# Ensembl/WiggleTools

Measured on AMD Instinct MI355X. Metric: genomic bp/s (whole node) for 'mean' over N BigWig tracks, higher is better.
Workload: dtype f64

## Files before the change

### include/wiggletools_amd.h

```cpp
#ifndef WIGGLETOOLS_AMD_H_
#define WIGGLETOOLS_AMD_H_

#include <stdint.h>
#include <stdio.h>

#ifdef __cplusplus
extern "C" {
#endif


typedef char wt_bool;

typedef struct wiggleIterator_st WiggleIterator;
typedef struct multiplexer_st Multiplexer;
typedef struct multiset_st Multiset;

struct wiggleIterator_st {
    char *chrom;
    int start;
    int finish;
    double value;
    void *valuePtr;
    wt_bool done;
    int strand;
// ... 343 lines not shown
    int32_t reserved;
} wtamd_pipe_config;

typedef struct {
    int64_t capacity;
    int64_t *seg_off;
    int32_t *start, *finish;
    float *value32;
    double *value64;
} wtamd_pipe_batch;

typedef struct {
    int64_t n_runs;
    const int32_t *start, *finish;
    const double *value;
    const double *tile;
    const uint8_t *inplay;
    int64_t covered_bp;
    int64_t n_intervals;
    int32_t integ_valid;
    int32_t reserved;
    double integ[6];
} wtamd_pipe_result;

typedef struct {
    int64_t batches, intervals, runs, covered_bp;
    int64_t h2d_bytes, d2h_bytes;
    double kernel_ms;
    double h2d_ms, d2h_ms;
    int32_t delta_batches;
    int32_t n_slots;
    double host_submit_ms;
    double host_wait_ms;
    int64_t bw_sections;
    double bw_decode_ms;
} wtamd_pipe_stats;

int wtamd_pipe_create(const wtamd_pipe_config *cfg, wtamd_pipe **out);
void wtamd_pipe_destroy(wtamd_pipe *);
int wtamd_pipe_acquire(wtamd_pipe *, wtamd_pipe_batch *out);
int wtamd_pipe_grow(wtamd_pipe *, int64_t used, int64_t min_capacity, int want_f64, wtamd_pipe_batch *out);
int wtamd_pipe_put_direct(wtamd_pipe *, int64_t at, int64_t count, const int32_t *start, const int32_t *finish,
                          const float *value);
int wtamd_pipe_submit(wtamd_pipe *, int value_is_f64, int32_t range_lo, int32_t range_hi);
int wtamd_pipe_cancel(wtamd_pipe *);
int wtamd_pipe_collect(wtamd_pipe *, wtamd_pipe_result *out);
int wtamd_pipe_release(wtamd_pipe *);
int wtamd_pipe_set_compress(wtamd_pipe *, int on);
int wtamd_pipe_set_integrate(wtamd_pipe *, int on);
int wtamd_pipe_integrate_modes(const wtamd_pipe *);
int wtamd_pipe_integrate_held(wtamd_pipe *, double *integ);
int wtamd_pipe_in_flight(const wtamd_pipe *);
int wtamd_pipe_get_stats(const wtamd_pipe *, wtamd_pipe_stats *out);

typedef struct {
    int64_t comp_off;
    uint32_t comp_size;
    int32_t track;
    uint32_t leaf_start, leaf_end;
} wtamd_bw_section;

typedef struct {
    uint32_t chrom_id;
    uint32_t chrom_len;
    int32_t box;
    int32_t compressed;
    int32_t clip_lo, clip_hi;
    int32_t first_section;
    int32_t n_sections;
    uint32_t plain_bytes;
    int32_t reserved;
} wtamd_bw_track;

int wtamd_pipe_bw_reserve(wtamd_pipe *, int64_t n_bytes, int64_t n_sections, uint8_t **bytes, wtamd_bw_section **sections);
int wtamd_pipe_submit_bw(wtamd_pipe *, int64_t n_bytes, int64_t n_sections, const wtamd_bw_track *tracks,
                         int32_t range_lo, int32_t range_hi);
int64_t wtamd_pipe_bw_fill_sections(const wtamd_pipe *);
unsigned wtamd_pipe_bw_error(const wtamd_pipe *);
int64_t wtamd_pipe_bw_redone(const wtamd_pipe *);

void *wtamd_host_alloc(size_t bytes);
void wtamd_host_free(void *);
void wtamd_pool_stats(int64_t out[6]);
void wtamd_pool_trim(void);


WiggleIterator *wtamd_ArrayReader(int n_chrom, const char *const *chrom_names, const int64_t *seg_off,
                                  const int32_t *start, const int32_t *finish, const float *value,
                                  double default_value);
WiggleIterator *wtamd_OverlappingArrayReader(int n_chrom, const char *const *chrom_names, const int64_t *seg_off,
                                             const int32_t *start, const int32_t *finish, const float *value,
                                             double default_value);
WiggleIterator *wtamd_CoverageIterator(WiggleIterator *child);
WiggleIterator *wtamd_RegionIterator(int op, WiggleIterator *source, WiggleIterator *mask);

Multiplexer *wtamd_ApplyMultiplexer(WiggleIterator *regions, const int *stats, int count, WiggleIterator *dataset, wt_bool strict);
Multiplexer *wtamd_ProfileMultiplexer(WiggleIterator *regions, int width, WiggleIterator *dataset);
WiggleIterator *wtamd_BinIterator(WiggleIterator *child, int width);
WiggleIterator *wtamd_SmoothIterator(WiggleIterator *child, int width);
typedef struct wtamd_histogram_st wtamd_Histogram;
wtamd_Histogram *wtamd_histogram(WiggleIterator **wigs, int count, int width);
void wtamd_normalize_histogram(wtamd_Histogram *hist);
void wtamd_print_histogram(wtamd_Histogram *hist, FILE *file);
int wtamd_histogram_width(const wtamd_Histogram *hist);
int wtamd_histogram_count(const wtamd_Histogram *hist);
const double *wtamd_histogram_row(const wtamd_Histogram *hist, int row);
void wtamd_histogram_range(const wtamd_Histogram *hist, double *lo_hi2);
void wtamd_destroy_histogram(wtamd_Histogram *hist);
WiggleIterator *wtamd_EnergyIntegrator(WiggleIterator *child, int wavelength);
int wtamd_EnergySpectrum(WiggleIterator *child, int n, const int *wavelengths, double *reim);
WiggleIterator *wtamd_TeeWiggleIterator(WiggleIterator *wi, FILE *out, wt_bool bedGraph, wt_bool holdFire);
void wtamd_toFile(WiggleIterator *wi, char *filename, wt_bool bedGraph, wt_bool holdFire);
void wtamd_toStdout(WiggleIterator *wi, wt_bool bedGraph, wt_bool holdFire);
Multiplexer *wtamd_TeeMultiplexer(Multiplexer *in, FILE *out, wt_bool bedGraph, wt_bool holdFire);
void wtamd_toStdoutMultiplexer(Multiplexer *in, wt_bool bedGraph, wt_bool holdFire);
Multiplexer *wtamd_PasteMultiplexer(Multiplexer *in, FILE *infile, FILE *outfile, wt_bool holdFire);
WiggleIterator *wtamd_BigWiggleReader(const char *path, int box);
int wtamd_BigWiggleReaders(int n, const char *const *paths, int box, WiggleIterator **out);
int wtamd_BigWiggleReader_close(WiggleIterator *wi);
WiggleIterator *wtamd_AUCIntegrator(WiggleIterator *wi);
WiggleIterator *wtamd_MeanIntegrator(WiggleIterator *wi);
WiggleIterator *wtamd_PearsonIntegrator(Multiplexer *multi);
WiggleIterator *wtamd_VarianceIntegrator(WiggleIterator *wi);
WiggleIterator *wtamd_StandardDeviationIntegrator(WiggleIterator *wi);
WiggleIterator *wtamd_CoefficientOfVariationIntegrator(WiggleIterator *wi);
WiggleIterator *wtamd_MaxIntegrator(WiggleIterator *wi);
WiggleIterator *wtamd_MinIntegrator(WiggleIterator *wi);
WiggleIterator *wtamd_SpanIntegrator(WiggleIterator *wi);
int64_t wtamd_iterator_next_block(WiggleIterator *wi, const char **chrom, const int32_t **start,
                                  const int32_t **finish, const double **value);
int wtamd_iterator_compress_output(WiggleIterator *wi, int on);
int wtamd_iterator_pipe_stats(WiggleIterator *wi, wtamd_pipe_stats *out);
int64_t wtamd_drain(WiggleIterator *wi, int64_t *covered_bp, double *value_sum);

typedef struct wtamd_bw wtamd_bw;
int wtamd_bw_open(const char *path, wtamd_bw **out);
void wtamd_bw_close(wtamd_bw *);
int wtamd_bw_n_chrom(const wtamd_bw *);
const char *wtamd_bw_chrom_name(const wtamd_bw *, int i);
uint32_t wtamd_bw_chrom_length(const wtamd_bw *, int i);
int64_t wtamd_bw_read_chrom(wtamd_bw *, const char *chrom, int box, int64_t capacity,
                            int32_t *start, int32_t *finish, float *value);

int64_t wtamd_bw_read_part(wtamd_bw *, const char *chrom, int box, int64_t *cursor, int max_blocks, int32_t lo0, int32_t hi0,
                           int64_t capacity, int32_t *start, int32_t *finish, float *value, int *last);

typedef struct bufferedReaderData_st BufferedReaderData;
void launchBufferedReader(void *(*readFileFunction)(void *), void *f_data, BufferedReaderData **buf_data);
wt_bool pushValuesToBuffer(BufferedReaderData *data, const char *chrom, int start, int finish, double value);
void endBufferedSignal(BufferedReaderData *data);
void killBufferedReader(BufferedReaderData *data);
void BufferedReaderPop(WiggleIterator *wi, BufferedReaderData *data);
int compare_chrom_lengths(const void *A, const void *B);
long long wtamd_bufreader_bulk_entries(void);
WiggleIterator *wtamd_BufferedArrayReader(int n_chrom, const char *const *chrom_names, const int64_t *seg_off,
                                          const int32_t *start, const int32_t *finish, const float *value,
                                          double default_value);

typedef struct wtamd_bw_writer wtamd_bw_writer;
int wtamd_bw_writer_open(const char *path, int n_chrom, const char *const *names, const uint32_t *lengths, int items_per_block,
                         int zlib_level, wtamd_bw_writer **out);
int wtamd_bw_writer_add(wtamd_bw_writer *, int chrom, int64_t n, const int32_t *start, const int32_t *finish, const float *value);
int64_t wtamd_bw_writer_close(wtamd_bw_writer *);
int wtamd_bw_writers_add_chrom(wtamd_bw_writer *const *writers, int n_tracks, int chrom, const int64_t *seg_off, const int32_t *start,
                               const int32_t *finish, const float *value, int threads);

// ... 13 lines not shown
```

### wiggletools_amd/csrc/wt_engine.hip

```cpp
#include <hip/hip_runtime.h>

#include <cstdio>
#include <thread>
#include <atomic>
#include <cstring>
#include <map>
#include <mutex>
#include <string>
#include <vector>

#include "wt_host.h"
#include "wt_trackset.h"
#include "wt_core.h"
#include "wt_plan.h"
#include "wt_kernels.h"
#include "wt_devscope.h"
#include "wt_pool.h"

#ifndef WT_INDEX_UNROLL
#define WT_INDEX_UNROLL 2
#endif
#define WT_INDEX_CHUNK (256 * 4 * WT_INDEX_UNROLL)
__global__ void __launch_bounds__(256) wt_index_kernel(const WtParams P, long long total, long long span) {
    const long long dev_total = P.seg_off[(long long) P.n_chrom * P.n_tracks];
// ... 169 lines not shown
    for (long long q = t; q < n_status; q += stride) status[q] = 0ull;
    for (long long q = t; q < n_counters; q += stride) counters[q] = 0ull;
    for (long long q = t; q < n_cro; q += stride) chrom_run_off[q] = 0;
}

__global__ void __launch_bounds__(256) wt_validate_kernel(const int32_t *start, const int32_t *finish, const int64_t *seg_off,
                                                           long long n_seg, long long total, unsigned long long *out) {
    const long long g = (long long) blockIdx.x * blockDim.x + threadIdx.x;
    if (g >= total) return;
    bool bad = finish[g] <= start[g];
    if (!bad && g > 0 && start[g] < finish[g - 1]) {
        long long lo = 0, hi = n_seg;
        while (hi - lo > 1) {
            const long long mid = (lo + hi) >> 1;
            if (seg_off[mid] <= g) lo = mid; else hi = mid;
        }
        bad = seg_off[lo] != g;
    }
    if (bad) {
        atomicAdd(&out[0], 1ull);
        atomicMin(&out[1], (unsigned long long) g);
    }
}

static thread_local std::string g_last_error;

int wt_fail(int code, const std::string &msg) {
    g_last_error = msg;
    return code;
}

template <class T>
static hipError_t wt_grow(T **p, int64_t *cap, int64_t need, bool *quiet) {
    if (*cap >= need && *p) return hipSuccess;
    int64_t c = *cap * 2;
    if (c < need) c = need;
    if (c < 1) c = 1;
    if (*p) {
        if (!*quiet) {
            const hipError_t eq = wt_pool_quiesce();
            if (eq != hipSuccess) return eq;
            *quiet = true;
        }
        (void) wt_dev_free(*p);
    }
    *p = nullptr; *cap = 0;
    const hipError_t e = wt_dev_alloc(p, sizeof(T) * (size_t) c);
    if (e == hipSuccess) *cap = c;
    return e;
}

static void wt_free_windows(WtWindows &w) {
    (void) wt_dev_free(w.d_tabs);
    (void) wt_dev_free(w.d_widx); (void) wt_dev_free(w.d_cidx); (void) wt_dev_free(w.d_status); (void) wt_dev_free(w.d_bad_list); (void) wt_dev_free(w.d_bad_goff);
    if (w.h_tab) wt_host_free(w.h_tab);
    if (w.ev_tab) (void) hipEventDestroy(w.ev_tab);
    w = WtWindows();
}

extern "C" {

const char *wtamd_last_error(void) { return g_last_error.c_str(); }
const char *wtamd_version(void) { return "wiggletools_amd 0.1 (gfx950)"; }

int wtamd_device_count(void) {
    int n = 0;
    if (hipGetDeviceCount(&n) != hipSuccess) return 0;
    return n;
}

__global__ void wt_warm_kernel(int *p) { if (p && threadIdx.x == 4096) *p = 0; }

static std::mutex g_warm_mu;
static std::thread *g_warm_thread = nullptr;
static bool g_warm_started = false;

extern "C++" void wt_warmup_join() {
    std::thread *t = nullptr;
    { std::lock_guard<std::mutex> lk(g_warm_mu); t = g_warm_thread; g_warm_thread = nullptr; }
    if (t) { t->join(); delete t; }
}

static std::atomic<int> g_device_chosen{-1};

void wtamd_warmup_async(void) {
    std::lock_guard<std::mutex> lk(g_warm_mu);
    if (g_warm_started || getenv("WTAMD_NO_WARMUP")) return;
    int n = 0, cur = -1;
    if (hipGetDeviceCount(&n) != hipSuccess || n <= 0) { (void) hipGetLastError(); return; }
    int ordinal = g_device_chosen.load();
    if (ordinal < 0 && hipGetDevice(&cur) == hipSuccess && (n == 1 || cur > 0)) ordinal = cur;
    if (ordinal < 0 || ordinal >= n) return;
    g_warm_started = true;
    g_warm_thread = new std::thread([ordinal] {
        if (hipSetDevice(ordinal) != hipSuccess) { (void) hipGetLastError(); return; }
        hipStream_t st[3] = {nullptr, nullptr, nullptr};
        for (auto &s : st)
            if (hipStreamCreateWithFlags(&s, hipStreamNonBlocking) != hipSuccess) s = nullptr;
        for (auto &s : st)
            if (s) hipLaunchKernelGGL(wt_warm_kernel, dim3(1), dim3(64), 0, s, (int *) nullptr);
        for (auto &s : st)
            if (s) { (void) hipStreamSynchronize(s); (void) hipStreamDestroy(s); }
        (void) hipGetLastError();
    });
    atexit(wt_warmup_join);
}

int wtamd_set_device(int ordinal) {
    wt_warmup_join();
    WT_HIP(hipSetDevice(ordinal));
    g_device_chosen.store(ordinal);
    return WTAMD_OK;
}

int wtamd_current_device(void) {
    int d = 0;
    if (hipGetDevice(&d) != hipSuccess) { (void) hipGetLastError(); return -1; }
    return d;
}

extern "C++" int wt_trackset_common(const wtamd_tracks *t, wtamd_trackset *ts) {
    if (!t || t->n_chrom < 0 || t->n_tracks <= 0 || !t->seg_off || !t->defaults)
        return wt_fail(WTAMD_ERR_ARG, "wtamd_trackset_create: bad tracks descriptor");
    if (wtamd_device_count() <= 0) return wt_fail(WTAMD_ERR_NODEVICE, "no HIP device visible");
    ts->n_chrom = t->n_chrom;
    ts->n_tracks = t->n_tracks;
    ts->value_f64 = t->value_is_f64 != 0;
    const int64_t n_seg = (int64_t) t->n_chrom * t->n_tracks;
    ts->seg_off.assign(t->seg_off, t->seg_off + n_seg + 1);
    for (int64_t s = 0; s < n_seg; s++)
        if (ts->seg_off[s + 1] < ts->seg_off[s]) return wt_fail(WTAMD_ERR_ARG, "seg_off not monotone");
    ts->n_intervals = ts->seg_off[n_seg] - ts->seg_off[0];
    if (ts->seg_off[0] != 0) return wt_fail(WTAMD_ERR_ARG, "seg_off[0] must be 0");
    ts->defaults.assign(t->defaults, t->defaults + t->n_tracks);
    if (t->range_lo && t->range_hi) {
        ts->range_lo.assign(t->range_lo, t->range_lo + t->n_chrom);
        ts->range_hi.assign(t->range_hi, t->range_hi + t->n_chrom);
    }
    ts->scratch_f32 = !ts->value_f64 && wt_defaults_fit_f32(ts->defaults.data(), ts->n_tracks);
    WT_HIP(hipGetDevice(&ts->device));
    hipDeviceProp_t prop;
    WT_HIP(hipGetDeviceProperties(&prop, ts->device));
    ts->num_cu = prop.multiProcessorCount;
    WT_HIP(wt_dev_alloc(&ts->d_seg_off, sizeof(int64_t) * (n_seg + 1)));
    WT_HIP(hipMemcpy(ts->d_seg_off, ts->seg_off.data(), sizeof(int64_t) * (n_seg + 1), hipMemcpyHostToDevice));
    WT_HIP(wt_dev_alloc(&ts->d_defaults, sizeof(double) * t->n_tracks));
    WT_HIP(hipMemcpy(ts->d_defaults, ts->defaults.data(), sizeof(double) * t->n_tracks, hipMemcpyHostToDevice));
    WT_HIP(wt_dev_alloc(&ts->d_counters, sizeof(unsigned long long) * WT_CTR_N));
    WT_HIP(wt_host_alloc((void **) &ts->h_counters, sizeof(unsigned long long) * WT_CTR_N));
    WT_HIP(wt_host_alloc((void **) &ts->h_debug, sizeof(unsigned long long) * 16));
    memset(ts->h_debug, 0, sizeof(unsigned long long) * 16);
    WT_HIP(wt_dev_alloc(&ts->d_chrom_run_off, sizeof(int64_t) * (t->n_chrom + 1)));
    WT_HIP(hipEventCreate(&ts->ev_i0));
    WT_HIP(hipEventCreate(&ts->ev_i1));
    WT_HIP(hipEventCreate(&ts->ev_r0));
    WT_HIP(hipEventCreate(&ts->ev_r1));
    return WTAMD_OK;
}

extern "C++" int wt_check_extents(wtamd_trackset *ts) {
    for (size_t q = 0; q < ts->last_finish.size(); q++)
        if (ts->seg_off[q + 1] > ts->seg_off[q] && ts->last_finish[q] > WTAMD_MAX_COORD) {
            const int64_t bad = ts->last_finish[q];
            return wt_fail(WTAMD_ERR_ARG, "run finish " + std::to_string(bad) + " above the supported maximum " +
                           std::to_string((long long) WTAMD_MAX_COORD) + " (2^31 - 65537)");
        }
    return WTAMD_OK;
}

static int wt_refresh_extents_device(wtamd_trackset *ts, hipStream_t s) {
    const int64_t n_seg = (int64_t) ts->n_chrom * ts->n_tracks;
    ts->first_start.assign(n_seg, 0);
    ts->last_finish.assign(n_seg, 0);
    if (n_seg > 0 && ts->n_intervals > 0) {
        const size_t bytes = sizeof(int32_t) * 2 * (size_t) n_seg;
        if (!ts->d_extents) WT_HIP(wt_dev_alloc(&ts->d_extents, bytes));
        if (!ts->h_extents) WT_HIP(wt_host_alloc((void **) &ts->h_extents, bytes));
        hipLaunchKernelGGL(wt_extents_kernel, dim3((unsigned) ((n_seg + 255) / 256)), dim3(256), 0, s,
                           ts->d_seg_off, ts->d_start, ts->d_finish, (long long) n_seg, ts->d_extents, ts->d_extents + n_seg);
        WT_HIP(hipGetLastError());
        WT_HIP(hipMemcpyAsync(ts->h_extents, ts->d_extents, bytes, hipMemcpyDeviceToHost, s));
        WT_HIP(hipStreamSynchronize(s));
        ts->first_start.assign(ts->h_extents, ts->h_extents + n_seg);
        ts->last_finish.assign(ts->h_extents + n_seg, ts->h_extents + 2 * n_seg);
    }
    return WTAMD_OK;
}

static int wt_create_host_impl(const wtamd_tracks *t, wtamd_trackset *ts) {
    int rc = wt_trackset_common(t, ts);
    if (rc != WTAMD_OK) return rc;
    ts->owns = true;
    const int64_t n = ts->n_intervals;
    const size_t vsz = ts->value_f64 ? 8 : 4;
    const int64_t n_alloc = n > 0 ? n : 1;
    WT_HIP(hipMalloc(&ts->d_start, sizeof(int32_t) * n_alloc));
    WT_HIP(hipMalloc(&ts->d_finish, sizeof(int32_t) * n_alloc));
    WT_HIP(hipMalloc(&ts->d_value, vsz * n_alloc));
    if (n > 0) {
        if (!t->start || !t->finish || !t->value) return wt_fail(WTAMD_ERR_ARG, "NULL arrays");
        WT_HIP(hipMemcpy(ts->d_start, t->start, sizeof(int32_t) * n, hipMemcpyHostToDevice));
        WT_HIP(hipMemcpy(ts->d_finish, t->finish, sizeof(int32_t) * n, hipMemcpyHostToDevice));
        WT_HIP(hipMemcpy(ts->d_value, t->value, vsz * n, hipMemcpyHostToDevice));
    }
    const int64_t n_seg = (int64_t) ts->n_chrom * ts->n_tracks;
    ts->first_start.assign(n_seg, 0);
    ts->last_finish.assign(n_seg, 0);
    for (int64_t s = 0; s < n_seg; s++)
        if (ts->seg_off[s + 1] > ts->seg_off[s]) {
            ts->first_start[s] = t->start[ts->seg_off[s]];
            ts->last_finish[s] = t->finish[ts->seg_off[s + 1] - 1];
        }
    return wt_check_extents(ts);
}

int wtamd_trackset_create_host(const wtamd_tracks *t, wtamd_trackset **out) {
    if (!out) return wt_fail(WTAMD_ERR_ARG, "out == NULL");
    wtamd_trackset *ts = new wtamd_trackset();
    const int rc = wt_create_host_impl(t, ts);
    if (rc != WTAMD_OK) { wtamd_trackset_destroy(ts); return rc; }
    *out = ts;
    return WTAMD_OK;
}

static int wt_create_device_impl(const wtamd_tracks *t, wtamd_trackset *ts) {
    int rc = wt_trackset_common(t, ts);
    if (rc != WTAMD_OK) return rc;
    ts->owns = false;
    ts->d_start = const_cast<int32_t *>(t->start);
    ts->d_finish = const_cast<int32_t *>(t->finish);
    ts->d_value = const_cast<void *>(t->value);
    rc = wt_refresh_extents_device(ts, nullptr);
    if (rc != WTAMD_OK) return rc;
    return wt_check_extents(ts);
}

int wtamd_trackset_create_device(const wtamd_tracks *t, wtamd_trackset **out) {
    if (!out) return wt_fail(WTAMD_ERR_ARG, "out == NULL");
    wtamd_trackset *ts = new wtamd_trackset();
    const int rc = wt_create_device_impl(t, ts);
    if (rc != WTAMD_OK) { wtamd_trackset_destroy(ts); return rc; }
    *out = ts;
    return WTAMD_OK;
}

void wtamd_trackset_destroy(wtamd_trackset *ts) {
    if (!ts) return;
    (void) wt_pool_quiesce();
    if (ts->owns) { (void) hipFree(ts->d_start); (void) hipFree(ts->d_finish); (void) hipFree(ts->d_value); }
    (void) wt_dev_free(ts->d_seg_off); (void) wt_dev_free(ts->d_defaults); (void) wt_dev_free(ts->d_counters); (void) wt_dev_free(ts->d_chrom_run_off);
    (void) wt_dev_free(ts->d_extents);
    (void) hipFree(ts->d_gscratch); (void) hipFree(ts->d_mwu_table);
    for (double *q : ts->mwu_retired) (void) hipFree(q);
    if (ts->h_counters) wt_host_free(ts->h_counters);
    if (ts->h_debug) wt_host_free(ts->h_debug);
    if (ts->h_extents) wt_host_free(ts->h_extents);
    for (auto &kv : ts->windows) wt_free_windows(kv.second);
    if (ts->ev_i0) (void) hipEventDestroy(ts->ev_i0);
    if (ts->ev_i1) (void) hipEventDestroy(ts->ev_i1);
    if (ts->ev_r0) (void) hipEventDestroy(ts->ev_r0);
    if (ts->ev_r1) (void) hipEventDestroy(ts->ev_r1);
    delete ts;
}

static int64_t wt_span(const wtamd_trackset *ts) {
    int64_t span = 0;
    for (int c = 0; c < ts->n_chrom; c++) {
        int64_t lo = INT64_MAX, hi = INT64_MIN;
        for (int i = 0; i < ts->n_tracks; i++) {
            const int64_t s = (int64_t) c * ts->n_tracks + i;
            if (ts->seg_off[s + 1] > ts->seg_off[s]) {
                lo = std::min<int64_t>(lo, ts->first_start[s]);
                hi = std::max<int64_t>(hi, ts->last_finish[s]);
            }
        }
        if (lo <= hi) span += hi - lo;
    }
    return span;
}

int64_t wtamd_trackset_max_runs(const wtamd_trackset *ts) {
    if (!ts) return 0;
    return std::min<int64_t>(2 * ts->n_intervals, wt_span(ts));
}

static int wt_get_windows(wtamd_trackset *ts, int W, WtWindows **out, hipStream_t s = nullptr) {
    WtWindows &w = ts->windows[W];
    *out = &w;
    if (w.tab_valid) return WTAMD_OK;
    wt_make_windows(ts->n_chrom, ts->n_tracks, ts->seg_off.data(), ts->first_start.data(), ts->last_finish.data(), W, w.tab,
                    ts->range_lo.empty() ? nullptr : ts->range_lo.data(),
                    ts->range_hi.empty() ? nullptr : ts->range_hi.data(), false);
    w.indexed = false;
    const int64_t nc = ts->n_chrom > 0 ? ts->n_chrom : 1;
    const int64_t nwin = w.tab.n_windows > 0 ? w.tab.n_windows : 1;
    const int64_t nwidx = (w.tab.n_rows > 0 ? w.tab.n_rows : 1) * (int64_t) ts->n_tracks;
    auto up8 = [](int64_t x) { return (x + 7) & ~(int64_t) 7; };
    bool quiet = false;
    if (w.cap_chrom < nc || w.cap_win < nwin || !w.d_tabs) {
        const int64_t cc = w.cap_chrom < nc ? std::max<int64_t>(nc, 2 * w.cap_chrom) : w.cap_chrom;
        const int64_t cw = w.cap_win < nwin ? std::max<int64_t>(nwin, 2 * w.cap_win) : w.cap_win;
        const int64_t o_cnwin = up8(4 * cc), o_chi = o_cnwin + up8(4 * cc), o_cfirst = o_chi + up8(4 * cc), o_win = o_cfirst + 8 * (cc + 1);
        const int64_t total = o_win + up8(4 * cw);
        if (w.d_tabs || w.d_status) { WT_HIP(wt_pool_quiesce()); quiet = true; }
        (void) wt_dev_free(w.d_tabs);
        w.d_tabs = nullptr; w.cap_tabs = 0;
        w.d_cbase = w.d_cnwin = w.d_chi = w.d_win_chrom = nullptr; w.d_cfirst = nullptr;
        if (w.cap_win < cw) { (void) wt_dev_free(w.d_status); w.d_status = nullptr; }
        w.cap_chrom = 0; w.cap_win = 0;
        WT_HIP(wt_dev_alloc(&w.d_tabs, (size_t) total));
        if (!w.d_status) WT_HIP(wt_dev_alloc(&w.d_status, sizeof(unsigned long long) * (size_t) cw));
        w.cap_tabs = total;
        w.d_cbase = (int32_t *) w.d_tabs; w.d_cnwin = (int32_t *) (w.d_tabs + o_cnwin); w.d_chi = (int32_t *) (w.d_tabs + o_chi);
        w.d_cfirst = (int64_t *) (w.d_tabs + o_cfirst); w.d_win_chrom = (int32_t *) (w.d_tabs + o_win);
        w.cap_chrom = cc; w.cap_win = cw;
    }
    WT_HIP(wt_grow(&w.d_widx, &w.cap_widx, nwidx, &quiet));
    WT_HIP(wt_grow(&w.d_cidx, &w.cap_cidx, ((w.tab.n_rows > 0 ? w.tab.n_rows : 1) + WT_ISEARCH_ROWS - 1) / WT_ISEARCH_ROWS * (int64_t) ts->n_tracks, &quiet));
    if (ts->n_chrom > 0) {
        if (ts->pipe_mode && ts->n_chrom != 1) return wt_fail(WTAMD_ERR_INTERNAL, "pipeline slots hold one chromosome");
        if (!w.ev_tab) WT_HIP(hipEventCreateWithFlags(&w.ev_tab, hipEventDisableTiming));
        if (w.tab_in_flight) { WT_HIP(hipEventSynchronize(w.ev_tab)); w.tab_in_flight = false; }
        const int64_t head = (char *) w.d_win_chrom - w.d_tabs;
        if (w.h_tab_bytes < head) {
            if (w.h_tab) wt_host_free(w.h_tab);
            w.h_tab = nullptr; w.h_tab_bytes = 0;
            WT_HIP(wt_host_alloc((void **) &w.h_tab, (size_t) head));
            w.h_tab_bytes = head;
        }
        const int64_t o_cfirst = (char *) w.d_cfirst - w.d_tabs;
        const int64_t used = o_cfirst + (int64_t) sizeof(int64_t) * (ts->n_chrom + 1);
        memset(w.h_tab, 0, (size_t) used);
        memcpy(w.h_tab + ((char *) w.d_cbase - w.d_tabs), w.tab.cbase.data(), sizeof(int32_t) * ts->n_chrom);
        memcpy(w.h_tab + ((char *) w.d_cnwin - w.d_tabs), w.tab.c_nwin.data(), sizeof(int32_t) * ts->n_chrom);
        memcpy(w.h_tab + ((char *) w.d_chi - w.d_tabs), w.tab.c_hi.data(), sizeof(int32_t) * ts->n_chrom);
        memcpy(w.h_tab + o_cfirst, w.tab.c_first_win.data(), sizeof(int64_t) * (ts->n_chrom + 1));
        WT_HIP(hipMemcpyAsync(w.d_tabs, w.h_tab, (size_t) used, hipMemcpyHostToDevice, s));
        WT_HIP(hipEventRecord(w.ev_tab, s));
        w.tab_in_flight = true;
        if (w.tab.n_windows > 0) {
            if (ts->n_chrom == 1) {
                WT_HIP(hipMemsetAsync(w.d_win_chrom, 0, sizeof(int32_t) * (size_t) w.tab.n_windows, s));
            } else {
                hipLaunchKernelGGL(wt_win_chrom_kernel, dim3((unsigned) ((w.tab.n_windows + 255) / 256)), dim3(256), 0, s,
                                   (const int64_t *) w.d_cfirst, ts->n_chrom, (long long) w.tab.n_windows, w.d_win_chrom);
                WT_HIP(hipGetLastError());
            }
        }
    }
    w.tab_valid = true;
    return WTAMD_OK;
}

static void wt_fill_params(const wtamd_trackset *ts, const WtWindows *w, const WtPlan &plan, WtParams &P) {
    memset(&P, 0, sizeof(P));
    P.start = ts->d_start; P.finish = ts->d_finish; P.value = ts->d_value;
    P.seg_off = ts->d_seg_off; P.defaults = ts->d_defaults;
    P.n_chrom = ts->n_chrom; P.n_tracks = ts->n_tracks; P.n_total = ts->n_intervals;
    P.cbase = w->d_cbase; P.c_nwin = w->d_cnwin; P.c_hi = w->d_chi; P.c_first_win = w->d_cfirst;
    P.n_windows = w->tab.n_windows; P.win_chrom = w->d_win_chrom; P.widx = w->d_widx;
    P.status = w->d_status; P.counters = ts->d_counters; P.debug = ts->h_debug;
    wt_plan_to_params(plan, P);
}

static int wt_build_index(wtamd_trackset *ts, WtWindows *w, const WtPlan &plan, hipStream_t s) {
    WtParams P;
    wt_fill_params(ts, w, plan, P);
    WT_HIP(hipEventRecord(ts->ev_i0, s));
    static const int mode = [] {
        const char *e = getenv("WTAMD_INDEX"), *c = getenv("WTAMD_INDEX_CHECK");
        if (c && atoi(c) > 0) return 2;
        return (e && !strcmp(e, "scan")) ? 1 : 0;
    }();
    const size_t n_widx = (size_t) w->tab.n_rows * ts->n_tracks;
    auto scan = [&](uint32_t *dst) -> int {
        WtParams Q = P;
        Q.widx = dst;
        WT_HIP(hipMemsetAsync(dst, 0, sizeof(uint32_t) * n_widx, s));
        if (ts->n_intervals > 0) {
            const long long total = ts->n_intervals;
            long long blocks = (total + WT_INDEX_CHUNK - 1) / WT_INDEX_CHUNK;
            const long long cap = (long long) ts->num_cu * 8;
            if (blocks > cap) blocks = cap;
            long long span = (total + blocks - 1) / blocks;
            span = (span + WT_INDEX_CHUNK - 1) / WT_INDEX_CHUNK * WT_INDEX_CHUNK;
            blocks = (total + span - 1) / span;
            hipLaunchKernelGGL(wt_index_kernel, dim3((unsigned) blocks), dim3(256), 0, s, Q, total, span);
            WT_HIP(hipGetLastError());
        }
        return WTAMD_OK;
    };
    auto search = [&](uint32_t *dst) -> int {
        WtParams Q = P;
        Q.widx = dst;
        const long long n_rows = w->tab.n_rows;
        if (n_rows > 0 && ts->n_tracks > 0) {
            const long long n_strips = (n_rows + WT_ISEARCH_ROWS - 1) / WT_ISEARCH_ROWS;
            if (w->cap_cidx < n_strips * ts->n_tracks) return wt_fail(WTAMD_ERR_INTERNAL, "coarse window index not allocated");
            hipLaunchKernelGGL(wt_index_coarse_kernel, dim3((unsigned) ((n_strips * ts->n_tracks + 255) / 256)), dim3(256), 0, s, Q, n_strips, w->d_cidx);
            WT_HIP(hipGetLastError());
            const dim3 grid((unsigned) n_strips, (unsigned) ((ts->n_tracks + WT_ISEARCH_TRACKS - 1) / WT_ISEARCH_TRACKS));
            hipLaunchKernelGGL(wt_index_search_kernel, grid, dim3(WT_ISEARCH_ROWS * WT_ISEARCH_TRACKS), 0, s, Q, n_rows, n_strips, (const uint32_t *) w->d_cidx);
            WT_HIP(hipGetLastError());
        }
        return WTAMD_OK;
    };
    if (mode == 1) {
        if (int rc = scan(w->d_widx)) return rc;
    } else {
        if (int rc = search(w->d_widx)) return rc;
    }
    if (mode == 2 && n_widx > 0) {
        uint32_t *other = nullptr;
        unsigned long long *d_diff = nullptr, h_diff = 0;
        WT_HIP(hipMalloc(&other, sizeof(uint32_t) * n_widx));
        WT_HIP(hipMalloc(&d_diff, sizeof(unsigned long long)));
        WT_HIP(hipMemsetAsync(d_diff, 0, sizeof(unsigned long long), s));
        if (int rc = scan(other)) return rc;
        hipLaunchKernelGGL(wt_index_compare_kernel, dim3((unsigned) ((n_widx + 255) / 256)), dim3(256), 0, s, w->d_widx, other, (long long) n_widx, d_diff);
        WT_HIP(hipMemcpyAsync(&h_diff, d_diff, sizeof(h_diff), hipMemcpyDeviceToHost, s));
        WT_HIP(hipStreamSynchronize(s));
        (void) hipFree(other); (void) hipFree(d_diff);
        if (h_diff) {
            fprintf(stderr, "wiggletools_amd: WTAMD_INDEX_CHECK: the searched window index differs from the scanned one in %llu of %zu entries\n", h_diff, n_widx);
            return wt_fail(WTAMD_ERR_INTERNAL, "window index check failed");
        }
    }
    WT_HIP(hipEventRecord(ts->ev_i1, s));
    ts->have_index_time = true;
    w->indexed = true;
    return WTAMD_OK;
}

static inline int wt_delta_class(int op) { return op == WT_OP_TTEST ? 1 : ((op == WT_OP_MAX || op == WT_OP_MIN) ? 2 : 0); }
static bool wt_wants_delta(const wtamd_trackset *ts, int op) {
    return !ts->delta_failed_[wt_delta_class(op)] && wt_delta_eligible(op, ts->value_f64, ts->n_tracks, ts->defaults.data());
}

static double wt_events_per_bp(const wtamd_trackset *ts) {
    const int64_t span = wt_span(ts);
    return span > 0 ? 1.25 * (double) ts->n_intervals / (double) span : 0.0;
}

static bool wt_mwu_few_ties(wtamd_trackset *ts, hipStream_t stream) {
    if (ts->mwu_few_ties >= 0) return ts->mwu_few_ties != 0;
    ts->mwu_few_ties = 0;
    if (hipStreamSynchronize(stream) != hipSuccess) { (void) hipGetLastError(); return false; }
    const int64_t n = ts->n_intervals;
    if (n < 1024 || ts->value_f64 || !ts->d_value) return false;
    const int64_t S = std::min<int64_t>(4096, n), stride = n / S;
    std::vector<uint32_t> v((size_t) S);
    if (hipMemcpy2D(v.data(), 4, ts->d_value, (size_t) stride * 4, 4, (size_t) S, hipMemcpyDeviceToHost) != hipSuccess) { (void) hipGetLastError(); return false; }
    std::sort(v.begin(), v.end());
    const int64_t distinct = (int64_t) (std::unique(v.begin(), v.end()) - v.begin());
    ts->mwu_few_ties = distinct * 100 >= S * 97 ? 1 : 0;
    return ts->mwu_few_ties != 0;
}

static bool wt_pick_plan(wtamd_trackset *ts, int op, int n_set0, WtPlan &plan, std::string &err, hipStream_t stream = nullptr) {
    static const int mwalk = getenv("WTAMD_MWALK") ? (atoi(getenv("WTAMD_MWALK")) != 0 ? 1 : 0) : -1;
    const bool walk = !getenv("WTAMD_NO_WALK");
    const bool mwu_walk = op == WT_OP_MWU && mwalk != 0 && !ts->value_f64 && walk && (mwalk == 1 || wt_mwu_few_ties(ts, stream));
    const double events_per_bp = (op == WT_OP_MEDIAN || op == WT_OP_MWU) ? wt_events_per_bp(ts) : 0.0;
    return wt_pick_general_plan(ts->n_tracks, op, ts->value_f64, ts->scratch_f32, n_set0, walk, mwu_walk, events_per_bp, plan, err);
}

static void wt_trackset_forget(wtamd_trackset *ts, bool delta_failed) {
    for (int q = 0; q < 3; q++) { ts->delta_verified_[q] = false; ts->delta_failed_[q] = delta_failed; ts->delta_n_bad_[q] = 0; }
    for (auto &kv : ts->windows) kv.second.indexed = false;
}

extern "C++" int wt_trackset_rebind(wtamd_trackset *ts, int64_t n, const int64_t *seg_off, int32_t range_lo, int32_t range_hi, bool value_f64,
                                    int32_t *d_start, int32_t *d_finish, void *d_value, bool delta_failed) {
    ts->n_intervals = n;
    ts->seg_off.assign(seg_off, seg_off + (int64_t) ts->n_chrom * ts->n_tracks + 1);
    ts->range_lo[0] = range_lo;
    ts->range_hi[0] = range_hi;
    ts->value_f64 = value_f64;
    ts->scratch_f32 = !ts->value_f64 && wt_defaults_fit_f32(ts->defaults.data(), ts->n_tracks);
    ts->d_start = d_start; ts->d_finish = d_finish; ts->d_value = d_value;
    wt_trackset_forget(ts, delta_failed);
    for (auto &kv : ts->windows) kv.second.tab_valid = false;
    return wt_check_extents(ts);
}

int wtamd_trackset_index(wtamd_trackset *ts, int op, void *stream) {
    if (!ts) return wt_fail(WTAMD_ERR_ARG, "ts == NULL");
    wt_trackset_forget(ts, false);
    ts->mwu_few_ties = -1;
    if (!ts->owns && !ts->pipe_mode) {
        int rce = wt_refresh_extents_device(ts, (hipStream_t) stream);
        if (rce != WTAMD_OK) return rce;
        rce = wt_check_extents(ts);
        if (rce != WTAMD_OK) return rce;
        for (auto &kv : ts->windows) kv.second.tab_valid = false;
    }
    WtPlan plan;
    std::string err;
    if (wt_wants_delta(ts, op)) wt_make_delta_plan_for(plan, ts->n_tracks, op);
    else if (!wt_pick_plan(ts, op, ts->n_tracks / 2, plan, err, (hipStream_t) stream)) return wt_fail(WTAMD_ERR_ARG, err);
    WtWindows *w = nullptr;
    int rc = wt_get_windows(ts, plan.W, &w, (hipStream_t) stream);
    if (rc != WTAMD_OK) return rc;
    return wt_build_index(ts, w, plan, (hipStream_t) stream);
}

extern "C++" int wt_check_desc(const wtamd_trackset *ts, const wtamd_reduce_desc *d) {
    if (!ts || !d) return wt_fail(WTAMD_ERR_ARG, "NULL argument");
    if (d->op < 0 || d->op >= WTAMD_OP_COUNT_) return wt_fail(WTAMD_ERR_ARG, "unknown op");
    if (d->op == WTAMD_OP_TTEST) {
        if (d->n_set0 < 3 || ts->n_tracks - d->n_set0 < 3)
            return wt_fail(WTAMD_ERR_ARG, "The t-test function only works for two sets with enough elements to compute variance");
    } else if (d->op == WTAMD_OP_MWU) {
        if (d->n_set0 < 1 || ts->n_tracks - d->n_set0 < 1)
            return wt_fail(WTAMD_ERR_ARG, "The Mann-Whitney U function only works for two non-empty sets");
    }
    return WTAMD_OK;
}

static int wt_reduce_plan(wtamd_trackset *ts, const WtPlan &plan, int op, uint32_t flags, int n_set0, wtamd_runs *runs,
                          double *d_tile, uint8_t *d_inplay, int64_t *n_runs, hipStream_t s);

extern "C++" int wt_launch_patch(wtamd_trackset *ts, int delta_W, int op, uint32_t flags, int n_set0, wtamd_runs *runs, long long n_bad,
                                 hipStream_t s) {
    WtPlan plan;
    std::string err;
    if (!wt_make_plan(ts->n_tracks, op, ts->scratch_f32, plan, err)) return wt_fail(WTAMD_ERR_INTERNAL, err);
    if (!wt_patch_compatible(plan, delta_W, ts->scratch_f32, ts->value_f64))
        return wt_fail(WTAMD_ERR_INTERNAL, "no general plan compatible with the difference-array windows (general W " + std::to_string(plan.W) + ", difference-array W " +
                       std::to_string(delta_W) + ", slab " + std::to_string((long long) plan.scratch_slab) + ", float staging " + std::to_string((int) ts->scratch_f32) + ", f64 values " +
                       std::to_string((int) ts->value_f64) + ")");
    WtWindows *dw = nullptr, *w = nullptr;
    int rc = wt_get_windows(ts, delta_W, &dw, s);
    if (rc != WTAMD_OK) return rc;
    rc = wt_get_windows(ts, plan.W, &w, s);
    if (rc != WTAMD_OK) return rc;
    WtLaunch L;
    WtParams &P = L.P;
    wt_fill_params(ts, w, plan, P);
    P.op = op; P.flags = flags; P.n_set0 = op == WT_OP_TTEST ? n_set0 : 0;
    P.capacity = runs->capacity;
    P.o_start = runs->start; P.o_finish = runs->finish; P.o_value = runs->value;
    P.chrom_run_off = runs->chrom_run_off ? runs->chrom_run_off : ts->d_chrom_run_off;
    L.T = plan.T; L.lds = plan.lds_bytes; L.stream = s; L.num_cu = ts->num_cu;
    WtPatchArgs Q;
    Q.bad_list = dw->d_bad_list; Q.bad_goff = dw->d_bad_goff;
    Q.n_bad = ts->d_counters + WT_CTR_DELTA_BAD;
    Q.d_win_chrom = dw->d_win_chrom; Q.d_c_first_win = dw->d_cfirst;
    Q.ratio = delta_W / plan.W;
    if (!wt_patch_launch(L, Q, op, plan.ppt, plan.n_chunks > 1, n_bad, !w->indexed))
        return wt_fail(WTAMD_ERR_INTERNAL, "no general plan compatible with the difference-array windows");
    if (L.err != hipSuccess) return wt_fail(WTAMD_ERR_HIP, std::string("patch kernel launch: ") + hipGetErrorString(L.err));
    WT_HIP(hipEventRecord(ts->ev_r1, s));
    ts->stats.patched_windows = (int32_t) n_bad;
    return WTAMD_OK;
}

static int wt_reduce_impl(wtamd_trackset *ts, int op, uint32_t flags, int n_set0, wtamd_runs *runs,
                          double *d_tile, uint8_t *d_inplay, int64_t *n_runs, hipStream_t s) {
    if (!runs || !runs->start || !runs->finish || !runs->value)
        return wt_fail(WTAMD_ERR_ARG, "wtamd_reduce: output arrays missing");
    WtPlan plan;
    std::string err;
    if (!d_tile && wt_wants_delta(ts, op)) {
        wt_make_delta_plan_for(plan, ts->n_tracks, op);
        const int dc = wt_delta_class(op);
        int64_t n_probe = 0;
        const bool probe = !ts->delta_verified_[dc];
        const int rc = wt_reduce_plan(ts, plan, op, flags, n_set0, runs, d_tile, d_inplay,
                                      (probe && !n_runs) ? &n_probe : n_runs, s);
        if (!probe) {
            if (ts->delta_n_bad_[dc] > 0 && (rc == WTAMD_OK || rc == WTAMD_ERR_CAPACITY)) {
                const int rp = wt_launch_patch(ts, plan.W, op, flags, n_set0, runs, ts->delta_n_bad_[dc], s);
                if (rp != WTAMD_OK) return rp;
                if (n_runs) WT_HIP(hipStreamSynchronize(s));
            }
            return rc;
        }
        if (rc != WTAMD_OK && rc != WTAMD_ERR_CAPACITY) return rc;
        const long long n_bad = (long long) ts->h_counters[WT_CTR_DELTA_BAD];
        if (n_bad == 0) { ts->delta_verified_[dc] = true; ts->delta_n_bad_[dc] = 0; return rc; }
        if (wt_few_enough_to_patch(n_bad, ts->stats.n_windows) && !getenv("WTAMD_NO_PATCH")) {
            const int rp = wt_launch_patch(ts, plan.W, op, flags, n_set0, runs, n_bad, s);
            if (rp == WTAMD_OK) {
                WT_HIP(hipStreamSynchronize(s));
                ts->delta_verified_[dc] = true;
                ts->delta_n_bad_[dc] = n_bad;
// ... 322 lines not shown
```

### wiggletools_amd/csrc/wt_trackset.h

```cpp
#ifndef WT_TRACKSET_H_
#define WT_TRACKSET_H_

#include <map>
#include <vector>

#include "wt_host.h"
#include "wt_plan.h"

struct WtWindows {
    WtPlan plan_geom;
    WtWindowTables tab;
    int32_t *d_cbase = nullptr, *d_cnwin = nullptr, *d_chi = nullptr, *d_win_chrom = nullptr;
    int64_t *d_cfirst = nullptr;
    uint32_t *d_widx = nullptr;
    uint32_t *d_cidx = nullptr;
    unsigned long long *d_status = nullptr;
    int32_t *d_bad_list = nullptr;
    long long *d_bad_goff = nullptr;
    bool indexed = false;
    int64_t cap_chrom = 0, cap_win = 0, cap_widx = 0, cap_bad = 0, cap_cidx = 0;
    bool tab_valid = false;
    char *h_tab = nullptr;
    int64_t h_tab_bytes = 0;
    hipEvent_t ev_tab = nullptr;
    bool tab_in_flight = false;
    char *d_tabs = nullptr;
    int64_t cap_tabs = 0;
};

struct wtamd_trackset {
    int n_chrom = 0, n_tracks = 0;
    bool value_f64 = false;
    bool owns = false;
    int64_t n_intervals = 0;
    std::vector<int64_t> seg_off;
    std::vector<double> defaults;
    std::vector<int32_t> first_start, last_finish;
    std::vector<int32_t> range_lo, range_hi;
    int32_t *d_start = nullptr, *d_finish = nullptr;
    void *d_value = nullptr;
    int64_t *d_seg_off = nullptr;
    double *d_defaults = nullptr;
    unsigned long long *d_counters = nullptr;
    unsigned long long *h_counters = nullptr;
    unsigned long long *h_debug = nullptr;
    int64_t *d_chrom_run_off = nullptr;
    int32_t *d_extents = nullptr, *h_extents = nullptr;
    char *d_gscratch = nullptr;
    size_t gscratch_bytes = 0;
    double *d_mwu_table = nullptr;
    int mwu_n1 = -1, mwu_n2 = -1, mwu_kmax = 0;
    int mwu_few_ties = -1;
    std::vector<double *> mwu_retired;
    std::map<int, WtWindows> windows;
    hipEvent_t ev_i0 = nullptr, ev_i1 = nullptr, ev_r0 = nullptr, ev_r1 = nullptr;
    bool have_index_time = false, have_reduce_time = false;
    wtamd_stats stats{};
    int device = 0;
    int num_cu = 256;
    bool scratch_f32 = false;
    bool delta_failed_[3] = {false, false, false};
    bool delta_verified_[3] = {false, false, false};
    long long delta_n_bad_[3] = {0, 0, 0};
    bool pipe_mode = false;
};

void wt_warmup_join();
int wt_trackset_common(const wtamd_tracks *t, wtamd_trackset *ts);
int wt_check_extents(wtamd_trackset *ts);
int wt_check_desc(const wtamd_trackset *ts, const wtamd_reduce_desc *d);

int wt_trackset_rebind(wtamd_trackset *ts, int64_t n, const int64_t *seg_off, int32_t range_lo, int32_t range_hi, bool value_f64,
                       int32_t *d_start, int32_t *d_finish, void *d_value, bool delta_failed);

int wt_reduce_enqueue(wtamd_trackset *ts, const wtamd_reduce_desc &desc, wtamd_runs *runs, double *d_tile, uint8_t *d_inplay,
                      hipStream_t s, bool *used_delta, int *delta_W);

int wt_launch_patch(wtamd_trackset *ts, int delta_W, int op, uint32_t flags, int n_set0, wtamd_runs *runs, long long n_bad,
                    hipStream_t s);

int wt_multiplex_device(wtamd_trackset *ts, uint32_t flags, wtamd_runs *runs, double *d_tile, uint8_t *d_inplay, int64_t *n_runs,
                        hipStream_t s);

#endif
```

Baseline: 50.45 billion.

## Speculatively build window index while device extents readback is in flight

The index build no longer blocks on a stream synchronize after the extents kernel. It records an event, picks the plan and enqueues the window and index build using the previous extents, then waits. If the fresh extents match the previous ones the speculative index is kept; otherwise it is invalidated and rebuilt. It also drops the single-chromosome memset shortcut in favour of always launching the win_chrom kernel, and adds counters for kept and redone indexes. When extents change, the speculative work is wasted and the index is built twice.

```diff
diff --git a/include/wiggletools_amd.h b/include/wiggletools_amd.h
--- a/include/wiggletools_amd.h
+++ b/include/wiggletools_amd.h
@@ -449,6 +449,7 @@
 void *wtamd_host_alloc(size_t bytes);
 void wtamd_host_free(void *);
 void wtamd_pool_stats(int64_t out[6]);
+void wtamd_index_stats(int64_t out[2]);
 void wtamd_pool_trim(void);
 
 
diff --git a/wiggletools_amd/csrc/wt_engine.hip b/wiggletools_amd/csrc/wt_engine.hip
--- a/wiggletools_amd/csrc/wt_engine.hip
+++ b/wiggletools_amd/csrc/wt_engine.hip
@@ -275,6 +275,7 @@
 }
 
 static std::atomic<int> g_device_chosen{-1};
+static std::atomic<int64_t> g_index_kept{0}, g_index_redone{0};
 
 void wtamd_warmup_async(void) {
     std::lock_guard<std::mutex> lk(g_warm_mu);
@@ -348,23 +349,29 @@
     WT_HIP(hipEventCreate(&ts->ev_i1));
     WT_HIP(hipEventCreate(&ts->ev_r0));
     WT_HIP(hipEventCreate(&ts->ev_r1));
-    return WTAMD_OK;
+    WT_HIP(hipEventCreateWithFlags(&ts->ev_ext, hipEventDisableTiming));
+    return WTAMD_OK;
+}
+
+static int64_t wt_first_bad_extent(const wtamd_trackset *ts) {
+    for (size_t q = 0; q < ts->last_finish.size(); q++)
+        if (ts->seg_off[q + 1] > ts->seg_off[q] && ts->last_finish[q] > WTAMD_MAX_COORD) return (int64_t) q;
+    return -1;
 }
 
 extern "C++" int wt_check_extents(wtamd_trackset *ts) {
-    for (size_t q = 0; q < ts->last_finish.size(); q++)
-        if (ts->seg_off[q + 1] > ts->seg_off[q] && ts->last_finish[q] > WTAMD_MAX_COORD) {
-            const int64_t bad = ts->last_finish[q];
-            return wt_fail(WTAMD_ERR_ARG, "run finish " + std::to_string(bad) + " above the supported maximum " +
-                           std::to_string((long long) WTAMD_MAX_COORD) + " (2^31 - 65537)");
-        }
-    return WTAMD_OK;
-}
-
-static int wt_refresh_extents_device(wtamd_trackset *ts, hipStream_t s) {
+    const int64_t q = wt_first_bad_extent(ts);
+    if (q >= 0) {
+        const int64_t bad = ts->last_finish[q];
+        return wt_fail(WTAMD_ERR_ARG, "run finish " + std::to_string(bad) + " above the supported maximum " +
+                       std::to_string((long long) WTAMD_MAX_COORD) + " (2^31 - 65537)");
+    }
+    return WTAMD_OK;
+}
+
+static int wt_extents_enqueue(wtamd_trackset *ts, hipStream_t s, bool *pending) {
     const int64_t n_seg = (int64_t) ts->n_chrom * ts->n_tracks;
-    ts->first_start.assign(n_seg, 0);
-    ts->last_finish.assign(n_seg, 0);
+    *pending = false;
     if (n_seg > 0 && ts->n_intervals > 0) {
         const size_t bytes = sizeof(int32_t) * 2 * (size_t) n_seg;
         if (!ts->d_extents) WT_HIP(wt_dev_alloc(&ts->d_extents, bytes));
@@ -373,10 +380,35 @@
                            ts->d_seg_off, ts->d_start, ts->d_finish, (long long) n_seg, ts->d_extents, ts->d_extents + n_seg);
         WT_HIP(hipGetLastError());
         WT_HIP(hipMemcpyAsync(ts->h_extents, ts->d_extents, bytes, hipMemcpyDeviceToHost, s));
-        WT_HIP(hipStreamSynchronize(s));
+        WT_HIP(hipEventRecord(ts->ev_ext, s));
+        *pending = true;
+    }
+    return WTAMD_OK;
+}
+
+static bool wt_extents_same(const wtamd_trackset *ts) {
+    const size_t n_seg = (size_t) ts->n_chrom * ts->n_tracks;
+    return ts->first_start.size() == n_seg && ts->last_finish.size() == n_seg &&
+           !memcmp(ts->h_extents, ts->first_start.data(), sizeof(int32_t) * n_seg) &&
+           !memcmp(ts->h_extents + n_seg, ts->last_finish.data(), sizeof(int32_t) * n_seg);
+}
+
+static void wt_extents_adopt(wtamd_trackset *ts, bool pending) {
+    const int64_t n_seg = (int64_t) ts->n_chrom * ts->n_tracks;
+    ts->first_start.assign(n_seg, 0);
+    ts->last_finish.assign(n_seg, 0);
+    if (pending) {
         ts->first_start.assign(ts->h_extents, ts->h_extents + n_seg);
         ts->last_finish.assign(ts->h_extents + n_seg, ts->h_extents + 2 * n_seg);
     }
+}
+
+static int wt_refresh_extents_device(wtamd_trackset *ts, hipStream_t s) {
+    bool pending = false;
+    const int rc = wt_extents_enqueue(ts, s, &pending);
+    if (rc != WTAMD_OK) return rc;
+    if (pending) WT_HIP(hipStreamSynchronize(s));
+    wt_extents_adopt(ts, pending);
     return WTAMD_OK;
 }
 
@@ -453,6 +485,7 @@
     if (ts->ev_i1) (void) hipEventDestroy(ts->ev_i1);
     if (ts->ev_r0) (void) hipEventDestroy(ts->ev_r0);
     if (ts->ev_r1) (void) hipEventDestroy(ts->ev_r1);
+    if (ts->ev_ext) (void) hipEventDestroy(ts->ev_ext);
     delete ts;
 }
 
@@ -532,13 +565,9 @@
         WT_HIP(hipEventRecord(w.ev_tab, s));
         w.tab_in_flight = true;
         if (w.tab.n_windows > 0) {
-            if (ts->n_chrom == 1) {
-                WT_HIP(hipMemsetAsync(w.d_win_chrom, 0, sizeof(int32_t) * (size_t) w.tab.n_windows, s));
-            } else {
-                hipLaunchKernelGGL(wt_win_chrom_kernel, dim3((unsigned) ((w.tab.n_windows + 255) / 256)), dim3(256), 0, s,
-                                   (const int64_t *) w.d_cfirst, ts->n_chrom, (long long) w.tab.n_windows, w.d_win_chrom);
-                WT_HIP(hipGetLastError());
-            }
+            hipLaunchKernelGGL(wt_win_chrom_kernel, dim3((unsigned) ((w.tab.n_windows + 255) / 256)), dim3(256), 0, s,
+                               (const int64_t *) w.d_cfirst, ts->n_chrom, (long long) w.tab.n_windows, w.d_win_chrom);
+            WT_HIP(hipGetLastError());
         }
     }
     w.tab_valid = true;
@@ -681,21 +710,53 @@
     if (!ts) return wt_fail(WTAMD_ERR_ARG, "ts == NULL");
     wt_trackset_forget(ts, false);
     ts->mwu_few_ties = -1;
-    if (!ts->owns && !ts->pipe_mode) {
-        int rce = wt_refresh_extents_device(ts, (hipStream_t) stream);
-        if (rce != WTAMD_OK) return rce;
-        rce = wt_check_extents(ts);
-        if (rce != WTAMD_OK) return rce;
-        for (auto &kv : ts->windows) kv.second.tab_valid = false;
-    }
+    const hipStream_t s = (hipStream_t) stream;
     WtPlan plan;
     std::string err;
-    if (wt_wants_delta(ts, op)) wt_make_delta_plan_for(plan, ts->n_tracks, op);
-    else if (!wt_pick_plan(ts, op, ts->n_tracks / 2, plan, err, (hipStream_t) stream)) return wt_fail(WTAMD_ERR_ARG, err);
+    auto pick = [&]() -> bool {
+        if (wt_wants_delta(ts, op)) { wt_make_delta_plan_for(plan, ts->n_tracks, op); return true; }
+        return wt_pick_plan(ts, op, ts->n_tracks / 2, plan, err, s);
+    };
+    if (!ts->owns && !ts->pipe_mode) {
+        static const bool speculate = [] { const char *e = getenv("WTAMD_INDEX_SPECULATE"); return !(e && !strcmp(e, "0")); }();
+        bool pending = false;
+        int rc = wt_extents_enqueue(ts, s, &pending);
+        if (rc != WTAMD_OK) return rc;
+        WtWindows *sw = nullptr;
+        bool spec_ok = false, spec_tab = false;
+        if (speculate && pending && wt_first_bad_extent(ts) < 0 && pick()) {
+            const auto it = ts->windows.find(plan.W);
+            spec_tab = it == ts->windows.end() || !it->second.tab_valid;
+            spec_ok = wt_get_windows(ts, plan.W, &sw, s) == WTAMD_OK && wt_build_index(ts, sw, plan, s) == WTAMD_OK;
+        }
+        if (pending) WT_HIP(hipEventSynchronize(ts->ev_ext));
+        if (spec_ok && wt_extents_same(ts)) {
+            g_index_kept.fetch_add(1, std::memory_order_relaxed);
+            return WTAMD_OK;
+        }
+        if (sw) {
+            g_index_redone.fetch_add(1, std::memory_order_relaxed);
+            sw->indexed = false;
+        }
+        wt_extents_adopt(ts, pending);
+        rc = wt_check_extents(ts);
+        if (rc != WTAMD_OK) {
+            if (sw && spec_tab) sw->tab_valid = false;
+            return rc;
+        }
+        for (auto &kv : ts->windows) kv.second.tab_valid = false;
+    }
+    if (!pick()) return wt_fail(WTAMD_ERR_ARG, err);
     WtWindows *w = nullptr;
-    int rc = wt_get_windows(ts, plan.W, &w, (hipStream_t) stream);
+    int rc = wt_get_windows(ts, plan.W, &w, s);
     if (rc != WTAMD_OK) return rc;
-    return wt_build_index(ts, w, plan, (hipStream_t) stream);
+    return wt_build_index(ts, w, plan, s);
+}
+
+void wtamd_index_stats(int64_t out[2]) {
+    if (!out) return;
+    out[0] = g_index_kept.load(std::memory_order_relaxed);
+    out[1] = g_index_redone.load(std::memory_order_relaxed);
 }
 
 extern "C++" int wt_check_desc(const wtamd_trackset *ts, const wtamd_reduce_desc *d) {
diff --git a/wiggletools_amd/csrc/wt_trackset.h b/wiggletools_amd/csrc/wt_trackset.h
--- a/wiggletools_amd/csrc/wt_trackset.h
+++ b/wiggletools_amd/csrc/wt_trackset.h
@@ -46,6 +46,7 @@
     unsigned long long *h_debug = nullptr;
     int64_t *d_chrom_run_off = nullptr;
     int32_t *d_extents = nullptr, *h_extents = nullptr;
+    hipEvent_t ev_ext = nullptr;
     char *d_gscratch = nullptr;
     size_t gscratch_bytes = 0;
     double *d_mwu_table = nullptr;
```

Result: no change. 50.34 billion (-0.2%).
